# empymod/emg3d

Hardware: AMD Instinct MI355X
Metric: Mcells/s per multigrid cycle (higher is better)
Workload: dtype c128

## Files before the change

emg3d_amd/_lib.py:

```python
import ctypes
import os

import numpy as np

_HERE = os.path.dirname(os.path.abspath(__file__))
LIB_PATH = os.environ.get("EMG3D_HIP_LIB") or os.path.join(_HERE, "libemg3d_hip.so")
LAB_PATH = os.path.join(_HERE, "libemg3d_hip_lab.so")

c_i64 = ctypes.c_int64
c_int = ctypes.c_int
c_vp = ctypes.c_void_p
c_double = ctypes.c_double
c_dp = ctypes.POINTER(ctypes.c_double)

ABI_VERSION = 116

SIGNATURES = {
    "emg3d_hip_version": (c_int, []),
    "emg3d_hip_device_count": (c_int, [ctypes.POINTER(c_int)]),
    "emg3d_hip_set_device": (c_int, [c_int]),
    "emg3d_hip_device_info": (c_int, [c_int, ctypes.c_char_p, ctypes.POINTER(c_i64), ctypes.POINTER(c_int)]),
    "emg3d_hip_mem_info": (c_int, [c_int, ctypes.POINTER(c_i64), ctypes.POINTER(c_i64)]),
    "emg3d_hip_release_cached": (c_i64, []),
    "emg3d_hip_cached_bytes": (c_i64, []),
    "emg3d_hip_cached_bytes_on": (c_i64, [c_int]),
    "emg3d_mg_placement": (c_int, [c_vp, c_int, ctypes.POINTER(c_int), ctypes.POINTER(c_int), ctypes.POINTER(ctypes.c_float)]),
    "emg3d_amat_x": (c_int, [c_int, c_i64, c_i64, c_i64, c_vp, c_vp, c_vp, c_vp, c_vp, c_vp, c_vp, c_vp, c_vp]),
    "emg3d_get_h_field": (c_int, [c_int, c_i64, c_i64, c_i64, c_vp, c_vp, c_vp, c_vp, c_vp, c_vp, c_double, c_double]),
    "emg3d_gauss_seidel": (c_int, [c_int, c_int, c_i64, c_i64, c_i64, c_vp, c_vp, c_vp, c_vp, c_vp, c_vp,
                                   c_vp, c_vp, c_vp, c_int, c_int]),
    "emg3d_restrict": (c_int, [c_int, c_i64, c_i64, c_i64, c_i64, c_i64, c_i64, c_vp, c_vp, c_vp, c_int]),
    "emg3d_restrict_weights": (c_int, [c_vp, c_vp, c_vp, c_i64, c_vp, c_vp, c_vp, c_i64, c_vp, c_vp, c_vp]),
    "emg3d_solve": (c_int, [c_int, c_vp, c_vp, c_i64]),
    "emg3d_blocks_to_amat": (c_int, [c_int, c_vp, c_vp, c_i64, c_vp, c_vp, c_vp, c_i64, c_i64]),
    "emg3d_prolongation": (c_int, [c_int, c_i64, c_i64, c_i64, c_vp, c_vp, c_vp, c_vp, c_vp, c_vp, c_int]),
    "emg3d_restrict_model": (c_int, [c_int, c_i64, c_i64, c_i64, c_vp, c_vp, c_int]),
    "emg3d_sweep_plan": (c_int, [c_int, c_i64, c_i64, c_i64, c_int, c_int, c_int, c_int, ctypes.c_char_p, ctypes.POINTER(c_i64)]),
    "emg3d_sweep_thm_zkeep": (c_int, [c_int, c_i64, c_i64, c_i64, c_int, c_int, c_int, c_int, ctypes.POINTER(c_i64)]),
    "emg3d_sweep_fuse_plan": (c_int, [c_int, c_i64, c_i64, c_i64, c_int, c_int, c_int, c_int, c_int, c_int, c_int, c_i64, ctypes.POINTER(c_i64),
                                      ctypes.POINTER(c_i64), c_i64]),
    "emg3d_mg_create": (c_int, [ctypes.POINTER(c_vp), c_int, c_i64, c_i64, c_i64, c_vp, c_vp, c_vp, c_vp,
                                c_vp, c_vp, c_vp, c_vp, c_int]),
    "emg3d_mg_destroy": (None, [c_vp]),
    "emg3d_mg_create_sv": (c_int, [ctypes.POINTER(c_vp), c_int, c_i64, c_i64, c_i64, c_vp, c_vp, c_vp, c_vp,
                                   c_vp, c_vp, c_vp, c_vp, c_double, c_double, c_int]),
    "emg3d_mg_create_vs": (c_int, [ctypes.POINTER(c_vp), c_int, c_i64, c_i64, c_i64, c_vp, c_vp, c_vp, c_vp,
                                   c_vp, c_vp, c_vp, c_vp, c_vp, c_double, c_double, c_int, c_int]),
    "emg3d_mg_create_vse": (c_int, [ctypes.POINTER(c_vp), c_int, c_i64, c_i64, c_i64, c_vp, c_vp, c_vp, c_vp,
                                    c_vp, c_vp, c_vp, c_vp, c_vp, c_vp, c_double, c_double, c_double, c_int, c_int]),
    "emg3d_mg_set_smu0_eps": (c_int, [c_vp, c_double, c_double, c_double]),
    "emg3d_mg_set_model": (c_int, [c_vp, c_int, c_vp, c_vp, c_vp]),
    "emg3d_mg_get_sigma": (c_int, [c_vp, c_int, c_vp]),
    "emg3d_mg_set_sfield_vector": (c_int, [c_vp, c_vp, c_double, c_double]),
    "emg3d_mg_set_sfield_dipole": (c_int, [c_vp, c_vp, c_vp, c_int, c_int, c_vp]),
    "emg3d_source_field": (c_int, [c_int, c_i64, c_i64, c_i64, c_vp, c_vp, c_vp, c_vp, c_vp, c_vp, c_int, c_vp, c_vp]),
# ... 52 lines not shown
    "emg3d_volume_average_adjoint": (c_int, [c_i64, c_i64, c_i64, c_vp, c_vp, c_vp, c_i64, c_i64, c_i64, c_vp, c_vp, c_vp, c_vp,
                                             c_vp, c_vp]),
    "emg3d_mg_set_model_grid": (c_int, [c_vp, c_i64, c_i64, c_i64, c_vp, c_vp, c_vp]),
    "emg3d_mg_set_regrid_factors": (c_int, [c_vp, c_vp, c_vp, c_vp, c_vp, c_vp, c_vp]),
    "emg3d_mg_grad_acc_get_model": (c_int, [c_vp, c_vp]),
    "emg3d_mg_grad_acc3_get_model": (c_int, [c_vp, c_vp, c_vp, c_vp]),
    "emg3d_interp3d_grid": (c_int, [c_int, c_i64, c_i64, c_i64, c_vp, c_vp, c_vp, c_vp, c_i64, c_vp, c_i64, c_vp, c_i64,
                                    c_vp, c_int, c_int, c_double, c_double, c_vp]),
    "emg3d_mg_set_batch": (c_int, [c_vp, c_int]),
    "emg3d_mg_get_batch": (c_int, [c_vp]),
    "emg3d_mg_select": (c_int, [c_vp, c_int]),
    "emg3d_mg_set_mask": (c_int, [c_vp, c_vp]),
    "emg3d_mg_residual_norm": (c_int, [c_vp, c_dp]),
    "emg3d_mg_sfield_norm": (c_int, [c_vp, c_dp]),
    "emg3d_mg_smooth": (c_int, [c_vp, c_int, c_int]),
    "emg3d_mg_begin": (c_int, [c_vp, c_int]),
    "emg3d_mg_set_smu0": (c_int, [c_vp, ctypes.c_double, ctypes.c_double]),
    "emg3d_mg_cycle": (c_int, [c_vp, c_int, c_int, c_dp]),
    "emg3d_mg_cycle_next": (c_int, [c_vp, c_int, c_int, c_int, c_int, c_dp]),
    "emg3d_mg_cycles": (c_int, [c_vp, c_int, c_vp, c_int, c_vp, c_int, c_vp]),
    "emg3d_mg_efield_devptr": (c_vp, [c_vp]),
    "emg3d_mg_sfield_devptr": (c_vp, [c_vp]),
    "emg3d_mg_stream": (c_vp, [c_vp]),
    "emg3d_mg_nE": (c_i64, [c_vp]),
    "emg3d_mg_sync": (c_int, [c_vp]),
    "emg3d_mg_device_bytes": (c_i64, [c_vp]),
    "emg3d_mg_time_sweep": (c_int, [c_vp, c_int, c_int, ctypes.POINTER(ctypes.c_float)]),
    "emg3d_mg_last_sweep_kernel": (c_int, [c_vp, ctypes.c_char_p]),
    "emg3d_mg_time_residual": (c_int, [c_vp, c_int, ctypes.POINTER(ctypes.c_float)]),
    "emg3d_mg_last_residual_kernel": (c_int, [c_vp, ctypes.c_char_p]),
# ... 131 lines not shown
    ranges = (c_i64 * cap)()
    check(load().emg3d_sweep_fuse_plan(dtype_code(dtype), int(vnC[0]), int(vnC[1]), int(vnC[2]), int(direction),
                                       1 if ordering == 'colour' else 0, int(nsys), int(cu_count), int(npass), int(own), int(max_seg), int(budget),
                                       info, ranges, cap), "emg3d_sweep_fuse_plan")
    out = {"fused": bool(info[0]), "axis": info[1], "nX": info[2], "own": info[3], "nslabs": info[4], "npass": info[5],
           "waves": info[6], "scratch_bytes": info[7], "slabs": []}
    if out["fused"]:
        per = 4 + 2 * int(npass)
        for k in range(info[4]):
            r = ranges[per * k:per * (k + 1)]
            out["slabs"].append({"own": (r[0], r[1]), "edges": (r[2], r[3]),
                                 "live": [(r[4 + 2 * p], r[5 + 2 * p]) for p in range(int(npass))]})
    return out


def rows_gram_plan(n_rows, n_cols):
    info = (c_i64 * 8)()
    check(load().emg3d_rows_gram_plan(int(n_rows), int(n_cols), info), "emg3d_rows_gram_plan")
    out = {"block": info[0], "kstep": info[1], "slab": info[2], "nslab": info[3], "nblocks": info[4], "njobs": info[5],
           "grid": info[6], "lds_bytes": info[7], "tile": 16, "jobs": []}
    rect = (c_i64 * 4)()
    for job in range(info[5]):
        check(load().emg3d_rows_gram_job(int(n_rows), job, rect), "emg3d_rows_gram_job")
        out["jobs"].append(tuple(rect))
    return out
```

emg3d_amd/csrc/emg3d_hip.hip:

```cpp
#include "../../include/emg3d_hip.h"

#include <cstring>
#include <new>

#include <chrono>
#include "mg.hpp"
#include "receivers.hpp"
#include "source.hpp"
#include "gradient.hpp"
#include "regrid.hpp"

#define EMG3D_HIP_VERSION EMG3D_HIP_ABI_VERSION

namespace {

template <class T>
MG<T>* as(emg3d_mg_t* mg) { return static_cast<MG<T>*>(reinterpret_cast<emg3d_mg*>(mg)); }

static int current_device() { int d = 0; if (hipGetDevice(&d) != hipSuccess) { (void)hipGetLastError(); d = 0; } return d; }

template <class T> static T scalar_of(double re, double im);
template <> double scalar_of<double>(double re, double) { return re; }
template <> c128 scalar_of<c128>(double re, double im) { return mk(re, im); }

// ... 524 lines not shown
    if (!f.fused || !ranges) return 0;
    const i64 per = 4 + 2 * (i64)npass;
    if (nranges < per * f.g.nslabs) return -2;
    for (int k = 0; k < f.g.nslabs; ++k) {
        int64_t* r = ranges + per * k;
        r[0] = fuse_x0(f.g, k); r[1] = fuse_x1(f.g, k);
        i64 a = -1, b = -1;
        for (int j = 0; j <= f.g.nX; ++j) if (fuse_owner(f.g, j) == k) { if (a < 0) a = j; b = j + 1; }
        r[2] = a; r[3] = b;
        for (int p = 0; p < npass; ++p) { r[4 + 2 * p] = fuse_lo(f.g, k, p); r[5 + 2 * p] = fuse_hi(f.g, k, p); }
    }
    return 0;
}

template <class T>
static int jvec_stage(MG<T>* m, const double* const hv[3], const double* dv[3]) {
    Level<T>& L = *m->lv0;
    double* stage = reinterpret_cast<double*>(L.r);
    const i64 n = L.nCells;
    int used = 0;
    for (int c = 0; c < 3; ++c) {
        dv[c] = nullptr;
        if (!hv[c]) continue;
        for (int q = 0; q < c; ++q) if (hv[q] == hv[c]) dv[c] = dv[q];
        if (dv[c]) continue;
        double* d = stage + (i64)used++ * n;
        HIP_TRY(hipMemcpyAsync(d, hv[c], (size_t)n * sizeof(double), hipMemcpyHostToDevice, m->stream));
        dv[c] = d;
    }
    return 0;
// ... 335 lines not shown
}

int emg3d_sweep_thm_zkeep(int dtype, int64_t nx, int64_t ny, int64_t nz, int dir, int order, int nsys, int cu_count, int64_t* info) {
    if (nx < 2 || ny < 2 || nz < 2 || dir < 1 || dir > 3 || order < 0 || order > 1 || nsys < 1 || nsys > 64 || !info) return -2;
    return dtype ? thm_zkeep_impl<c128>(nx, ny, nz, dir, order, nsys, cu_count, info)
                 : thm_zkeep_impl<double>(nx, ny, nz, dir, order, nsys, cu_count, info);
}

int emg3d_sweep_fuse_plan(int dtype, int64_t nx, int64_t ny, int64_t nz, int dir, int order, int nsys, int cu_count, int npass, int own,
                          int max_seg, int64_t budget, int64_t* info, int64_t* ranges, int64_t nranges) {
    if (nx < 2 || ny < 2 || nz < 2 || dir < 1 || dir > 3 || order < 0 || order > 1 || nsys < 1 || nsys > 64 || npass < 0 || !info) return -2;
    return dtype ? fuse_plan_impl<c128>(nx, ny, nz, dir, order, nsys, cu_count, npass, own, max_seg, budget, info, ranges, nranges)
                 : fuse_plan_impl<double>(nx, ny, nz, dir, order, nsys, cu_count, npass, own, max_seg, budget, info, ranges, nranges);
}

int emg3d_mg_create(emg3d_mg_t** out, int dtype, int64_t nx, int64_t ny, int64_t nz, const double* hx,
                    const double* hy, const double* hz, const double* origin, const void* eta_x,
                    const void* eta_y, const void* eta_z, const double* zeta, int device) {
    if (!out) return -1;
    return dtype ? create_impl<c128>(out, 1, nx, ny, nz, hx, hy, hz, origin, eta_x, eta_y, eta_z, zeta, device)
                 : create_impl<double>(out, 0, nx, ny, nz, hx, hy, hz, origin, eta_x, eta_y, eta_z, zeta, device);
}

int emg3d_mg_create_sv(emg3d_mg_t** out, int dtype, int64_t nx, int64_t ny, int64_t nz, const double* hx,
                       const double* hy, const double* hz, const double* origin, const double* sv_x,
                       const double* sv_y, const double* sv_z, const double* zeta, double smu0_re,
                       double smu0_im, int device) {
    if (!out || !sv_x) return -1;
    return dtype ? create_impl<c128>(out, 1, nx, ny, nz, hx, hy, hz, origin, sv_x, sv_y, sv_z, zeta, device, true, smu0_re, smu0_im)
                 : create_impl<double>(out, 0, nx, ny, nz, hx, hy, hz, origin, sv_x, sv_y, sv_z, zeta, device, true, smu0_re, smu0_im);
// ... 818 lines not shown
```

emg3d_amd/csrc/mg.hpp:

```cpp
#pragma once
#include <algorithm>
#include <cmath>
#include <cstdlib>
#include <cstring>
#include <map>
#include <memory>
#include <mutex>
#include <chrono>
#include <vector>

#include "common.hpp"
#include "smooth.hpp"
#include "stencil.hpp"
#include "gradient.hpp"
#include "regrid.hpp"
#include "rows.hpp"
#include "smooth_qpl.hpp"
#include "smooth_qc.hpp"
#include "smooth_thm.hpp"
#include "smooth_tha.hpp"
#include "sweep_launch.hpp"
#include "sweep_plan.hpp"

template <class T>
// ... 15 lines not shown
    T *eT = nullptr, *sT = nullptr;
    T* etaT[3] = {nullptr, nullptr, nullptr};
    double* zetaT = nullptr;
    bool sT_valid = false;
    FieldLayout flT;
    CellLayout clT;
    T *eW[2] = {nullptr, nullptr}, *sW[2] = {nullptr, nullptr};
    double* zetaW[2] = {nullptr, nullptr};
    bool sW_valid[2] = {false, false};
    int e_home = 0;
    T* fac[3] = {nullptr, nullptr, nullptr};
    void* qd[3][4] = {{nullptr, nullptr, nullptr, nullptr}, {nullptr, nullptr, nullptr, nullptr}, {nullptr, nullptr, nullptr, nullptr}};
    unsigned qdn[3][4] = {{0, 0, 0, 0}, {0, 0, 0, 0}, {0, 0, 0, 0}};
    T* fz[3] = {nullptr, nullptr, nullptr};
    i64 fz_n[3] = {0, 0, 0};
    FusePlan fuse[3];
    int fuse_key[3] = {-1, -1, -1};
    std::vector<int> passes[3];
    i64 fac_lines[3] = {0, 0, 0};
    i64 fac_mid[3] = {0, 0, 0};
    int fac_kind[3] = {0, 0, 0};
    SweepPlan plan[3];
    int plan_key[3] = {-1, -1, -1};
};

struct Transfer {
    int sc = -1;
    int co[3] = {0, 0, 0};
    double* w[3][3] = {{nullptr, nullptr, nullptr}, {nullptr, nullptr, nullptr}, {nullptr, nullptr, nullptr}};
    int* pidx[3] = {nullptr, nullptr, nullptr};
// ... 1141 lines not shown
        a.xcd = xcd_map;
        a.tile = q_tile;
        {
            const int ax[3] = {a.L, a.P, a.Q};
            a.rs.ihL = a.ih[a.L]; a.rs.ihP = a.ih[a.P]; a.rs.ihQ = a.ih[a.Q];
            a.rs.hL = a.h[a.L]; a.rs.hP = a.h[a.P]; a.rs.hQ = a.h[a.Q];
            a.rs.nL = (unsigned)a.nC[a.L]; a.rs.slot0 = 0;
            a.rs.nP = (unsigned)a.nC[a.P]; a.rs.nQ = (unsigned)a.nC[a.Q];
            a.rs.csL = (unsigned)a.cl.st[a.L]; a.rs.csP = (unsigned)a.cl.st[a.P]; a.rs.csQ = (unsigned)a.cl.st[a.Q];
            for (int c = 0; c < 3; ++c) {
                a.rs.off[c] = (unsigned)a.fl.off[ax[c]];
                for (int d = 0; d < 3; ++d) a.rs.st[c][d] = (unsigned)a.fl.st[ax[c]][ax[d]];
            }
        }
        a.qd = nullptr; a.qdn = 0;
        a.fe = nullptr; a.fnE = 0; a.fax = a.fnX = a.fown = a.fns = a.fnp = 0; a.fseq = 0;
        for (int c = 0; c < 4; ++c) { a.fqd[c] = nullptr; a.fqdn[c] = 0; }
        a.qpl = P.NW; a.qM = P.M; a.seg = P.seg; a.qlpw = 0;
        a.tha = P.helpers;
        a.mode = 0; a.cP = a.cQ = 0; a.cntA = a.cntB = 0; a.t = a.jQ0 = a.cnt = 0;
        a.bt = sweep ? batch(L) : Batch();
    }

    void ensure_factor(Level<T>& L, int dir) {
        const SweepPlan& P = plan(L, dir);
        if (P.xt) ensure_transposed_model(L);
        if (L.fac[dir]) return;
        L.fac_lines[dir] = (L.nC[dir == 0 ? 1 : 0] - 1) * (L.nC[dir == 2 ? 1 : 2] - 1);
        L.fac[dir] = dalloc<T>(L.fac_lines[dir] * P.fac_entries);
        L.fac_mid[dir] = P.mid;
        L.fac_kind[dir] = P.fac_kind;
// ... 283 lines not shown
        L.passes[dir].clear();
        if (order != 1) return F;
        colour_passes(L, dir, nu, L.passes[dir]);
        const std::vector<int>& seq = L.passes[dir];
        plan(L, dir);
        F = plan_fuse(knobs, SweepShape{{L.nC[0], L.nC[1], L.nC[2]}, (int)sizeof(T)}, dir, (int)seq.size());
        if (!F.fused) return F;
        for (int c : seq) if (!L.qd[dir][c]) { F.fused = false; return F; }
        const i64 need = (i64)nsys * F.g.nslabs * L.nE;
        if (L.fz_n[dir] < need) {
            T* z = try_alloc<T>(need);
            if (!z) { F.fused = false; return F; }
            if (L.fz[dir]) release(L.fz[dir]);
            L.fz[dir] = z; L.fz_n[dir] = need;
        }
        return F;
    }
    void smooth_fused(Level<T>& L, int dir, const SweepPlan& P, const FusePlan& F, const std::vector<int>& seq, const LineArgs<T>& a) {
        LineArgs<T> b = a;
        b.mode = 0; b.xcd = 0;
        b.fe = L.fz[dir]; b.fnE = L.nE; b.fax = F.axis;
        b.fnX = F.g.nX; b.fown = F.g.own; b.fns = F.g.nslabs; b.fnp = F.g.npass;
        b.fseq = 0;
        for (int p = 0; p < F.g.npass; ++p) b.fseq |= (unsigned long long)seq[(size_t)p] << (4 * p);
        for (int c = 0; c < 4; ++c) { b.fqd[c] = L.qd[dir][c]; b.fqdn[c] = L.qd[dir][c] ? L.qdn[dir][c] : 0u; }
        if (log_launches) fprintf(stderr, "[sweep] nC %lld %lld %lld L %d lines %lld kernel %s split %d fused passes %d slabs %d own %d\n", (long long)a.nC[0],
                                  (long long)a.nC[1], (long long)a.nC[2], a.L, (long long)a.nLinesTot, P.name, a.split, F.g.npass, F.g.nslabs, F.g.own);
        memcpy(sweep_name, P.name, sizeof sweep_name);
        if (broken) return;
        qpl_fused_launch<T>(P.family == SweepFamily::qpl_chain, bgrid((unsigned)F.g.nslabs), stream, b);
        ScatterArgs sa;
        sa.nE = L.nE; sa.g = F.g;
        int Pa, Qa;
        sweep_axes(dir, Pa, Qa);
        sa.ax = F.axis ? Qa : Pa;
        for (int c = 0; c < 3; ++c) {
            sa.off[c] = L.fl.off[c];
            sa.d0[c] = (unsigned)((c == 0) ? L.nC[0] : L.nC[0] + 1); sa.d1[c] = (unsigned)((c == 1) ? L.nC[1] : L.nC[1] + 1);
        }
        hipLaunchKernelGGL(k_scatter_slabs<T>, dim3((unsigned)((L.nE + EMG_BLOCK - 1) / EMG_BLOCK), (unsigned)nsys), dim3(EMG_BLOCK), 0, stream,
                           a.e, (const T*)L.fz[dir], sa, a.bt);
    }

    void smooth_line(Level<T>& L, int dir, int nu, bool conv_in = true, bool conv_out = true) {
        if (nu <= 0) return;
        ensure_factor(L, dir);
        ensure_qdesc(L, dir);
        const FusePlan& F = ensure_fuse(L, dir, nu);
        if (dry) { prepare_work(L, dir); return; }
        if (conv_in) to_work(L, dir);
        ensure_sflags(L, dir);
        LineArgs<T> a;
        line_args(L, dir, a, true);
        const SweepPlan& P = plan(L, dir);
        const i64 nP = L.nC[a.P], nQ = L.nC[a.Q];
        const i64 nB[2] = {(nQ - 0) / 2, (nQ - 1) / 2};
        if (order == 1) {
            if (F.fused) smooth_fused(L, dir, P, F, L.passes[dir], a);
            else for (int c : L.passes[dir]) {
                a.mode = 0; a.cP = c & 1; a.cQ = c >> 1;
                a.cntA = a.nA[a.cP]; a.cntB = nB[a.cQ];
                a.rs.slot0 = (unsigned)a.base[c];
                a.qd = L.qd[dir][c]; a.qdn = (L.qd[dir][c] ? L.qdn[dir][c] : 0u);
                launch_sweep(P, a, a.cntA * a.cntB);
            }
            nu = 0;
        }
        int iback = 0;
        for (int it = 0; it < nu; ++it) {
            iback = 1 - iback;
            {
                const i64 tmin = 3, tmax = (nP - 1) + 2 * (nQ - 1);
                if (lex_loop && a.qpl && a.qM == 1 && a.seg <= 16) {
// ... 57 lines not shown
                                       dim3(EMG_LINE_BLOCK), 0, stream, a);
                }
            }
        }
        if (hl) convert_field(L, L.eW[1], L.e, 1, true);
        check_launch();
    }

    void smoothing(Level<T>& L, int nu, int lr_dir) {
        const int lr = current_lr_dir(lr_dir, L.nC);
        if (lr == 0) smooth_point(L, nu);
        int dirs[3], nd = 0;
        if (lr == 1 || lr == 5 || lr == 6 || lr == 7) dirs[nd++] = 0;
        if (lr == 2 || lr == 4 || lr == 6 || lr == 7) dirs[nd++] = 1;
        if (lr == 3 || lr == 4 || lr == 5 || lr == 7) dirs[nd++] = 2;
        for (int k = 0; k < nd; ++k) {
            const bool in = (k == 0) || work_id(L, dirs[k - 1]) != work_id(L, dirs[k]);
            const bool out = (k == nd - 1) || work_id(L, dirs[k + 1]) != work_id(L, dirs[k]);
            smooth_line(L, dirs[k], nu, in, out);
        }
    }

    void residual(Level<T>& L, int mode, int slot) {
        ResidualArgs<T> a;
        for (int q = 0; q < 3; ++q) { a.nC[q] = L.nC[q]; a.eta[q] = L.eta[q]; a.h[q] = L.h[q]; a.ih[q] = L.ih[q]; }
        a.fl = L.fl; a.r = L.r; a.s = L.s; a.e = L.e; a.zeta = L.zeta; a.bt = batch(L);
        if (!dry && L.e_home == 1) {
            if (!L.sW_valid[1]) { convert_field(L, L.sW[1], L.s, 1, true); L.sW_valid[1] = true; }
            a.e = L.eW[1]; a.s = L.sW[1]; a.xs = 1;
        }
        const i64 plane = (L.nC[0] + 1) * (L.nC[1] + 1);
        const i64 cells = L.nC[0] * L.nC[1] * L.nC[2];
        const int kz = cells < res_zm_min ? 1 : res_kz ? res_kz : (cells * nsys >= ((i64)8 << 20) ? 8 : 4);
        const i64 nNz = L.nC[2] + 1;
// ... 209 lines not shown
```

emg3d_amd/csrc/smooth.hpp:

```cpp
#pragma once
#include "common.hpp"

#define EMG_LINE_BLOCK 64

template <class T>
struct LineArgs {
    int L, P, Q;
    i64 nC[3];
    FieldLayout fl;
    CellLayout cl;
    T* e;
    const T* s;
    const T* eta[3];
    const double* zeta;
    const double* h[3];
    const double* ih[3];
    int split;
    i64 mid;
    int xcd;
    int tile;
    struct Resolved {
        const double *ihL, *ihP, *ihQ;
        const double *hL, *hP, *hQ;
        unsigned nL, csL, csP, csQ;
// ... 2 lines not shown
        unsigned off[3], st[3][3];
    } rs;
    Batch bt;
    int qm;
    int qpl;
    int qM, seg;
    const unsigned char* sflag;
    int zsep;
    int qlpw;
    int tha;
    int fcomp;
    T* fac;
    const void* qd;
    unsigned qdn;
    T* fe;
    i64 fnE;
    int fax, fnX, fown, fns, fnp;
    unsigned long long fseq;
    const void* fqd[4];
    unsigned fqdn[4];
    i64 nLinesTot;
    i64 base[4];
    i64 nA[2];
    i64 nB2[2];
    int mode;
    int cP, cQ;
    i64 cntA, cntB;
    i64 t, jQ0, cnt;
};

// ... 1174 lines not shown
```

emg3d_amd/csrc/smooth_qpl.hpp:

```cpp
#pragma once
#include "smooth.hpp"
#include "sweep_plan.hpp"


template <int K>
__device__ __forceinline__ double quad_bcast(double v) {
    constexpr int ctrl = K | (K << 2) | (K << 4) | (K << 6);
    int lo = __double2loint(v), hi = __double2hiint(v);
    lo = __builtin_amdgcn_update_dpp(0, lo, ctrl, 0xf, 0xf, false);
    hi = __builtin_amdgcn_update_dpp(0, hi, ctrl, 0xf, 0xf, false);
    return __hiloint2double(hi, lo);
}
template <int K>
__device__ __forceinline__ c128 quad_bcast(c128 v) { return mk(quad_bcast<K>(v.re), quad_bcast<K>(v.im)); }
__device__ __forceinline__ double quad_sum(double v) {
    int lo = __double2loint(v), hi = __double2hiint(v);
    double o = __hiloint2double(__builtin_amdgcn_update_dpp(0, hi, 0xb1, 0xf, 0xf, false),
                                __builtin_amdgcn_update_dpp(0, lo, 0xb1, 0xf, 0xf, false));
    v += o;
    lo = __double2loint(v); hi = __double2hiint(v);
    o = __hiloint2double(__builtin_amdgcn_update_dpp(0, hi, 0x4e, 0xf, 0xf, false),
                         __builtin_amdgcn_update_dpp(0, lo, 0x4e, 0xf, 0xf, false));
    return v + o;
}
// ... 450 lines not shown
        }
        if (j > 0) {
            const double ar = (r == 0) ? av[j][0] : (r == 1) ? av[j][1] : (r == 2) ? av[j][2] : av[j][3];
            const double dr = (r == 0) ? dv[j][0] : (r == 1) ? dv[j][1] : (r == 2) ? dv[j][2] : dv[j][3];
            T vr = x0 * ar;
            cmac(vr, xr, dr);
            v[0] = quad_bcast<0>(vr); v[1] = quad_bcast<1>(vr); v[2] = quad_bcast<2>(vr); v[3] = quad_bcast<3>(vr);
        }
    }
    QPL_TS(6);
    };

    if constexpr (FZ) {
        const FuseGeom g{a.fnX, a.fown, a.fns, a.fnp};
        const int k = (int)wg;
        {
            T* __restrict__ dst = ebase;
            const T* __restrict__ src = a.e + boff_;
            const int ra = fuse_lo(g, k, 0) - 1, rb = fuse_hi(g, k, 0) + 1;
            const int X = a.fax ? 2 : 1;
            const u32 nO = a.fax ? a.rs.nP : a.rs.nQ;
#pragma unroll
            for (int c = 0; c < 3; ++c) {
                const u32 dL = a.rs.nL + (c != 0 ? 1u : 0u), dX = (u32)g.nX + (c != X ? 1u : 0u), dO = nO + ((c == 0 || c == X) ? 1u : 0u);
                const int rbc = rb < (int)dX - 1 ? rb : (int)dX - 1;
                if (rbc < ra) continue;
                const u32 w = (u32)(rbc - ra + 1);
                const u32 stL = a.rs.st[c][0], stX = a.fax ? a.rs.st[c][2] : a.rs.st[c][1], stO = a.fax ? a.rs.st[c][1] : a.rs.st[c][2];
                const bool xf = stX < stL;
                const u32 n0 = xf ? w : dL, n1 = xf ? dL : w, tot = n0 * n1 * dO;
                for (u32 idx = (u32)tid; idx < tot; idx += 64u * NW) {
                    const u32 t = idx / n0, i0 = idx - t * n0, i2 = t / n1, i1 = t - i2 * n1;
                    const u32 iX = (u32)ra + (xf ? i0 : i1), iL = xf ? i1 : i0;
                    const u32 off = a.rs.off[c] + iL * stL + iX * stX + i2 * stO;
                    dst[off] = src[off];
                }
            }
        }
        __threadfence_block();
        __syncthreads();
        const u32 lslot = (u32)(quad >> lseg), wslot0 = (u32)(((tid >> 6) * 16) >> lseg);
        for (int p = 0; p < g.npass; ++p) {
            const int c = (int)((a.fseq >> (4 * p)) & 3ull);
            const int cP = c & 1, cQ = c >> 1;
            const u32 cA = (u32)a.nA[cP], cB = (u32)a.nB2[cQ];
            const int cX = a.fax ? cQ : cP;
            const u32 qa = (u32)(fuse_lo(g, k, p) - cX) >> 1, qb = (u32)(fuse_hi(g, k, p) + 1 - cX) >> 1;
            const u32 nx = qb > qa ? qb - qa : 0u;
            const u32 nloc = nx * (a.fax ? cA : cB);
            qd_ = a.fqd[c]; qdn_ = a.fqdn[c];
            for (u32 base = 0; base < nloc; base += (u32)lpg) {
                if (base + wslot0 < nloc) {
                    const u32 m = base + lslot;
                    const bool lv = m < nloc;
                    const u32 mm = lv ? m : base + wslot0;
                    u32 qq, bq;
                    if (a.fax == 0) { bq = mm / nx; qq = qa + (mm - bq * nx); }
                    else { const u32 t = mm / cA; qq = mm - t * cA; bq = qa + t; }
                    const u32 gl = bq * cA + qq;
                    tix = ((gl >> (4 - lseg)) << 6) + ((((gl & ((16u >> lseg) - 1u)) << lseg) + (u32)ch) << 2) + (u32)r;
                    one(lv ? 0u : 1u, 1u, 0u, 0u);
                }
            }
            __threadfence_block();
            __syncthreads();
        }
    } else if constexpr (!HL) {
        one((u32)wg * (u32)lpg + (u32)(quad >> lseg), (u32)((a.mode == 0) ? a.cntA * a.cntB : a.cnt), (u32)a.t, (u32)a.jQ0);
#ifdef EMG3D_LAB
        if ((a.tile & 512) && blockIdx.x == 0 && threadIdx.x == 0) {
            asm volatile("s_waitcnt vmcnt(0)" ::: "memory");
            const long long tend = (long long)__builtin_readcyclecounter();
            printf("[qpl<%d,%d> seg %d lines %lld] args %lld loads issued %lld loads in + coefficients %lld forward %lld backward %lld stores issued %lld stores done %lld (cycles after entry)\n",
                   NW, M, seg, (long long)(a.cntA * a.cntB), qts[1] - qts[0], qts[2] - qts[0], qts[3] - qts[0], qts[4] - qts[0], qts[5] - qts[0], qts[6] - qts[0], tend - qts[0]);
        }
#endif
    } else {
        const int nPm = (int)a.rs.nP - 1, nQm = (int)a.rs.nQ - 1;
        const int tmin = (int)a.t, tmax = (int)a.jQ0;
        for (int th = tmin; th <= tmax; ++th) {
            const int tt = a.cnt ? tmax - (th - tmin) : th;
// ... 16 lines not shown
```

emg3d_amd/csrc/sweep_plan.hpp:

```cpp
#pragma once
#include <algorithm>
#include <cstdint>
#include <cstdio>
#include <cstdlib>

typedef int64_t i64;

#ifndef LAB_ENV
#ifdef EMG3D_LAB
inline long long lab_env_(const char* name, long long def) { const char* v = getenv(name); return v ? atoll(v) : def; }
inline int lab_env_ch_(const char* name) { const char* v = getenv(name); return v ? v[0] : 0; }
#define LAB_ENV(name, def) lab_env_(name, (long long)(def))
#define LAB_ENV_CH(name) lab_env_ch_(name)
#else
#define LAB_ENV(name, def) ((long long)(def))
#define LAB_ENV_CH(name) 0
#endif
#endif

constexpr int SWEEP_THA_LPW = 8, SWEEP_THA_RING = 8, SWEEP_THA_MAX_DYN_LDS = 140 * 1024, SWEEP_THA_STATIC_LDS = 18 * 1024;
inline i64 sweep_tha_lds_bytes(i64 nL, int tsize) {
    return (2 * SWEEP_THA_RING * 5 + 2 * ((nL + 1) / 2 + 2)) * (5 * SWEEP_THA_LPW) * (i64)tsize;
}

// ... 22 lines not shown
    int q_stages = (int)LAB_ENV("EMG3D_Q_STAGES", 0);
    int q_lpw = (int)LAB_ENV("EMG3D_Q_LPW", 0);
    int q_big_lab = (int)LAB_ENV("EMG3D_Q_BIG", 0);
    int use_qpl = (int)LAB_ENV("EMG3D_QPL", 7);
    i64 qpl_min_nl = LAB_ENV("EMG3D_QPL_MIN", 2);
    i64 qpl_max_nl = LAB_ENV("EMG3D_QPL_MAX_NL", 64);
    i64 qpl_m2_min = LAB_ENV("EMG3D_QPL_M2", 32);
    int qpl_chain_seg = (int)LAB_ENV("EMG3D_QPL_CHAIN", 4);
    i64 qpl_few_lines_env = LAB_ENV("EMG3D_QPL_FEW", 0);
    i64 qpl_max_lines = LAB_ENV("EMG3D_QPL_MAX", (i64)1 << 40);
    int use_qdesc = (int)LAB_ENV("EMG3D_QDESC", 1);
    i64 qdesc_max_threads_env = LAB_ENV("EMG3D_QDESC_MAX", 0);
    int fuse_max_seg = (int)LAB_ENV("EMG3D_QPL_FUSE", 4);
    i64 fuse_own = LAB_ENV("EMG3D_QPL_FUSE_W", 0);
    i64 fuse_max_bytes = LAB_ENV("EMG3D_QPL_FUSE_BYTES", (i64)64 << 20);
    int use_tha = (int)LAB_ENV("EMG3D_THA", 3);
    i64 tha_min_nl = LAB_ENV("EMG3D_THA_MIN", 33), tha_mid_nl = LAB_ENV("EMG3D_THA_MID", 64), tha_min_lines_env = LAB_ENV("EMG3D_THA_MIN_LINES", 0);
    i64 tha_max_nl = LAB_ENV("EMG3D_THA_MAX", 128);
    i64 tha_big_max_lines_env = LAB_ENV("EMG3D_THA_BIG_LINES", 0);
    int tha_split = (int)LAB_ENV("EMG3D_THA_SPLIT", 0);

    i64 q_min_lines() const { return q_min_lines_env > 0 ? q_min_lines_env : 8 * simds; }
    i64 twist_max_lines() const { return twist_max_lines_env > 0 ? twist_max_lines_env : q_min_lines(); }
    i64 qpl_few_lines() const { return qpl_few_lines_env > 0 ? qpl_few_lines_env : simds; }
    i64 qdesc_max_threads() const { return qdesc_max_threads_env > 0 ? qdesc_max_threads_env : (9000 * simds + 1023) / 1024; }
    i64 tha_min_lines() const { return tha_min_lines_env > 0 ? tha_min_lines_env : (1100 * simds + 1023) / 1024; }
    i64 tha_big_max_lines() const { return tha_big_max_lines_env > 0 ? tha_big_max_lines_env : (i64)SWEEP_THA_LPW * (simds / 4); }
};

struct SweepShape {
// ... 178 lines not shown
    if (P.family != SweepFamily::thm || !K.thm_lds_granted || K.thm_zkeep == 0) return 0;
    const i64 n = G.nC[dir], m = (n - 1) / 2, half = std::max(m, n - m - 2);
    const i64 room = K.lds_limit - sweep_thm_static_lds(P.inst_lpw, G.tsize);
    i64 kz = std::min(half, room / sweep_thm_keep_step_bytes(P.inst_lpw, G.tsize));
    if (K.thm_zkeep > 0) kz = std::min(kz, K.thm_zkeep);
    return std::max<i64>(kz, 0);
}

constexpr int SWEEP_FUSE_MAX_PASSES = 16;
struct FuseGeom { int nX, own, nslabs, npass; };
SWEEP_HD inline int fuse_x0(const FuseGeom& g, int k) { return 1 + k * g.own; }
SWEEP_HD inline int fuse_x1(const FuseGeom& g, int k) { const int x = 1 + (k + 1) * g.own; return (k == g.nslabs - 1 || x > g.nX) ? g.nX : x; }
SWEEP_HD inline int fuse_lo(const FuseGeom& g, int k, int p) { const int v = fuse_x0(g, k) - (g.npass - 1 - p); return v < 1 ? 1 : v; }
SWEEP_HD inline int fuse_hi(const FuseGeom& g, int k, int p) { const int v = fuse_x1(g, k) + (g.npass - 1 - p); return v > g.nX - 1 ? g.nX - 1 : v; }
SWEEP_HD inline int fuse_owner(const FuseGeom& g, int j) { const int k = j <= 0 ? 0 : (j - 1) / g.own; return k > g.nslabs - 1 ? g.nslabs - 1 : k; }

struct FusePlan {
    bool fused = false;
    int axis = 0;
    int nw = 0;
    FuseGeom g = {0, 0, 0, 0};
    i64 scratch_bytes = 0;
};
inline void sweep_axes(int dir, int& P, int& Q) { P = dir == 0 ? 1 : 0; Q = dir == 2 ? 1 : 2; }
inline FusePlan plan_fuse(const SweepKnobs& K, const SweepShape& G, int dir, int npass) {
    FusePlan f;
    const SweepPlan p = plan_sweep(K, G, dir);
    if (K.order != 1 || (p.family != SweepFamily::qpl && p.family != SweepFamily::qpl_chain) || p.NW != 1 || p.M != 1 || !p.qdesc) return f;
    if (p.seg > K.fuse_max_seg || p.seg > 8 || npass < 3 || npass > SWEEP_FUSE_MAX_PASSES) return f;
#ifndef EMG3D_LAB
    if (p.family != SweepFamily::qpl_chain) return f;
#endif
    int P, Q;
    sweep_axes(dir, P, Q);
    f.axis = G.nC[Q] > G.nC[P] ? 1 : 0;
    const i64 nX = G.nC[f.axis ? Q : P];
    if (nX < 2 || nX > (1 << 20)) return f;
    i64 own = K.fuse_own > 0 ? K.fuse_own : 2;
    own = std::min<i64>(own, nX - 1);
    f.g.nX = (int)nX; f.g.own = (int)own; f.g.nslabs = (int)((nX - 1 + own - 1) / own); f.g.npass = npass;
    f.nw = p.family == SweepFamily::qpl_chain ? 8 : 4;
    f.scratch_bytes = (i64)K.nsys * f.g.nslabs * G.edges() * (i64)G.tsize;
    f.fused = f.scratch_bytes <= K.fuse_max_bytes;
    return f;
}
```

emg3d_amd/solver.py:

```python
import ctypes
import itertools
import time
from dataclasses import dataclass
from datetime import datetime, timedelta

import warnings

import numpy as np
import scipy.sparse.linalg as ssl

from emg3d_amd import _lib, core, fields, meshes, models

__all__ = ['solve', 'multigrid', 'krylov', 'smoothing', 'restriction', 'prolongation',
           'residual', 'MGParameters', 'DeviceMG', 'FrequencyHandles']

ORDERINGS = {'lex': 0, 'colour': 1, 'color': 1}


def _cells(a, dtype=np.float64):
    return np.ascontiguousarray(np.asarray(a, dtype=dtype).ravel(order='F'))


class DeviceMG:

# ... 511 lines not shown
        n = self.nsys
        out = np.empty(n, dtype=np.float64)
        _lib.check(fn(self._h, *args, out.ctypes.data_as(ctypes.POINTER(ctypes.c_double))), name)
        return float(out[0]) if n == 1 else out

    def residual_norm(self):
        return self._norms(self._lib.emg3d_mg_residual_norm, "emg3d_mg_residual_norm")

    def sfield_norm(self):
        v = ctypes.c_double()
        _lib.check(self._lib.emg3d_mg_sfield_norm(self._h, ctypes.byref(v)), "emg3d_mg_sfield_norm")
        return v.value

    def smooth(self, nu, lr_dir):
        _lib.check(self._lib.emg3d_mg_smooth(self._h, int(nu), int(lr_dir)), "emg3d_mg_smooth")

    def begin(self, sc_dir):
        _lib.check(self._lib.emg3d_mg_begin(self._h, int(sc_dir)), "emg3d_mg_begin")

    def cycle(self, sc_dir, lr_dir, nxt=None):
        if nxt is not None:
            return self._norms(self._lib.emg3d_mg_cycle_next, "emg3d_mg_cycle_next", int(sc_dir), int(lr_dir),
                               int(nxt[0]), int(nxt[1]))
        return self._norms(self._lib.emg3d_mg_cycle, "emg3d_mg_cycle", int(sc_dir), int(lr_dir))

    def cycles(self, n, sc_cycle, lr_cycle):
        sc = np.ascontiguousarray(sc_cycle, dtype=np.int32)
        lr = np.ascontiguousarray(lr_cycle, dtype=np.int32)
        ns = self.nsys
        out = np.empty(n * ns, dtype=np.float64)
# ... 1776 lines not shown
```

include/emg3d_hip.h:

```cpp
#ifndef EMG3D_HIP_H
#define EMG3D_HIP_H

#include <stdint.h>

#ifdef __cplusplus
extern "C" {
#endif

#define EMG3D_HIP_ABI_VERSION 116
int emg3d_hip_version(void);
int emg3d_hip_device_count(int* count);
int emg3d_hip_set_device(int device);
int emg3d_hip_device_info(int device, char* name, int64_t* total_mem, int* cu_count);
int emg3d_hip_mem_info(int device, int64_t* free_bytes, int64_t* total_bytes);

int64_t emg3d_hip_release_cached(void);
int64_t emg3d_hip_cached_bytes(void);
int64_t emg3d_hip_cached_bytes_on(int device);


int emg3d_amat_x(int dtype, int64_t nx, int64_t ny, int64_t nz, void* r, const void* e,
                 const void* eta_x, const void* eta_y, const void* eta_z, const double* zeta,
                 const double* hx, const double* hy, const double* hz);

// ... 20 lines not shown

int emg3d_prolongation(int dtype, int64_t nx, int64_t ny, int64_t nz, const double* hx,
                       const double* hy, const double* hz, const double* origin, void* e,
                       const void* ce, int sc_dir);

int emg3d_restrict_model(int is_complex, int64_t nx, int64_t ny, int64_t nz, void* cparam,
                         const void* param, int sc_dir);

int emg3d_sweep_plan(int dtype, int64_t nx, int64_t ny, int64_t nz, int dir, int order, int nsys, int cu_count, char* name,
                     int64_t* info);

int emg3d_sweep_thm_zkeep(int dtype, int64_t nx, int64_t ny, int64_t nz, int dir, int order, int nsys, int cu_count, int64_t* info);

int emg3d_sweep_fuse_plan(int dtype, int64_t nx, int64_t ny, int64_t nz, int dir, int order, int nsys, int cu_count, int npass, int own,
                          int max_seg, int64_t budget, int64_t* info, int64_t* ranges, int64_t nranges);

typedef struct emg3d_mg emg3d_mg_t;

int emg3d_mg_create(emg3d_mg_t** out, int dtype, int64_t nx, int64_t ny, int64_t nz,
                    const double* hx, const double* hy, const double* hz, const double* origin,
                    const void* eta_x, const void* eta_y, const void* eta_z, const double* zeta,
                    int device);
int emg3d_mg_create_sv(emg3d_mg_t** out, int dtype, int64_t nx, int64_t ny, int64_t nz, const double* hx,
                       const double* hy, const double* hz, const double* origin, const double* sv_x,
                       const double* sv_y, const double* sv_z, const double* zeta, double smu0_re,
                       double smu0_im, int device);

int emg3d_mg_create_vs(emg3d_mg_t** out, int dtype, int64_t nx, int64_t ny, int64_t nz, const double* hx,
                       const double* hy, const double* hz, const double* origin, const double* sigma_x,
                       const double* sigma_y, const double* sigma_z, const double* vol, const double* zeta,
// ... 99 lines not shown
int emg3d_mg_grad_acc3_get_model(emg3d_mg_t* mg, double* out_x, double* out_y, double* out_z);
int emg3d_interp3d_grid(int dtype, int64_t nx, int64_t ny, int64_t nz, const double* px, const double* py, const double* pz,
                        const void* values, int64_t mx, const double* xi_x, int64_t my, const double* xi_y, int64_t mz,
                        const double* xi_z, int method, int has_fill, double fill_value, double cval, void* out);

int emg3d_mg_set_batch(emg3d_mg_t* mg, int n);
int emg3d_mg_get_batch(emg3d_mg_t* mg);
int emg3d_mg_select(emg3d_mg_t* mg, int b);
int emg3d_mg_set_mask(emg3d_mg_t* mg, const int* active);

int emg3d_mg_residual_norm(emg3d_mg_t* mg, double* l2);
int emg3d_mg_sfield_norm(emg3d_mg_t* mg, double* l2);

int emg3d_mg_smooth(emg3d_mg_t* mg, int nu, int lr_dir);

int emg3d_mg_set_smu0(emg3d_mg_t* mg, double smu0_re, double smu0_im);
int emg3d_mg_set_smu0_eps(emg3d_mg_t* mg, double smu0_re, double smu0_im, double seps0);

int emg3d_mg_set_model(emg3d_mg_t* mg, int map, const double* p_x, const double* p_y, const double* p_z);
int emg3d_mg_get_sigma(emg3d_mg_t* mg, int comp, double* out);

int emg3d_mg_begin(emg3d_mg_t* mg, int sc_dir);

int emg3d_mg_cycle(emg3d_mg_t* mg, int sc_dir, int lr_dir, double* l2);
int emg3d_mg_cycle_next(emg3d_mg_t* mg, int sc_dir, int lr_dir, int next_sc_dir, int next_lr_dir, double* l2);
int emg3d_mg_set_trace(emg3d_mg_t* mg, int on);
int emg3d_mg_get_trace(emg3d_mg_t* mg, int max_recs, int64_t* recs, double* norms, int* count);
int emg3d_mg_prepare(emg3d_mg_t* mg, int sc_dir, int lr_dir);

int emg3d_mg_cycles(emg3d_mg_t* mg, int ncycles, const int* sc_cycle, int n_sc, const int* lr_cycle,
// ... 41 lines not shown
```

Before: 259.2.

## Pair consecutive fused line sweeps through a ping-pong array to skip scatter pass

When two consecutive fused line-relaxation directions work on the same array, the first fused kernel now writes its owned slab region directly into a ping-pong buffer, and the second reads from that buffer and writes back into the field. This skips the separate scatter kernel launch and the scratch-to-field copy for each paired call. It costs an extra field-sized allocation and an extra owned-range copy inside the fused kernel. It also adds a planning helper and debug/introspection entry points.

```diff
diff --git a/emg3d_amd/_lib.py b/emg3d_amd/_lib.py
--- a/emg3d_amd/_lib.py
+++ b/emg3d_amd/_lib.py
@@ -13,7 +13,7 @@
 c_double = ctypes.c_double
 c_dp = ctypes.POINTER(ctypes.c_double)
 
-ABI_VERSION = 116
+ABI_VERSION = 117
 
 SIGNATURES = {
     "emg3d_hip_version": (c_int, []),
@@ -39,6 +39,8 @@
     "emg3d_sweep_thm_zkeep": (c_int, [c_int, c_i64, c_i64, c_i64, c_int, c_int, c_int, c_int, ctypes.POINTER(c_i64)]),
     "emg3d_sweep_fuse_plan": (c_int, [c_int, c_i64, c_i64, c_i64, c_int, c_int, c_int, c_int, c_int, c_int, c_int, c_i64, ctypes.POINTER(c_i64),
                                       ctypes.POINTER(c_i64), c_i64]),
+    "emg3d_sweep_fuse_pairs": (c_int, [c_int, ctypes.POINTER(c_int), ctypes.POINTER(c_int), c_int, c_int, ctypes.POINTER(c_int)]),
+    "emg3d_sweep_fuse_owned": (c_int, [c_int, c_int, c_int, ctypes.POINTER(c_i64)]),
     "emg3d_mg_create": (c_int, [ctypes.POINTER(c_vp), c_int, c_i64, c_i64, c_i64, c_vp, c_vp, c_vp, c_vp,
                                 c_vp, c_vp, c_vp, c_vp, c_int]),
     "emg3d_mg_destroy": (None, [c_vp]),
@@ -121,6 +123,7 @@
     "emg3d_mg_residual_norm": (c_int, [c_vp, c_dp]),
     "emg3d_mg_sfield_norm": (c_int, [c_vp, c_dp]),
     "emg3d_mg_smooth": (c_int, [c_vp, c_int, c_int]),
+    "emg3d_mg_fuse_roles": (c_int, [c_vp, c_int, c_int, ctypes.POINTER(c_int), ctypes.POINTER(c_int)]),
     "emg3d_mg_begin": (c_int, [c_vp, c_int]),
     "emg3d_mg_set_smu0": (c_int, [c_vp, ctypes.c_double, ctypes.c_double]),
     "emg3d_mg_cycle": (c_int, [c_vp, c_int, c_int, c_dp]),
@@ -282,6 +285,20 @@
     return out
 
 
+def sweep_fuse_pairs(fused, work_id, write_back=None, have_pingpong=True):
+    n = len(fused)
+    f, w, role = (c_int * max(n, 1))(*[int(bool(v)) for v in fused]), (c_int * max(n, 1))(*[int(v) for v in work_id]), (c_int * max(n, 1))()
+    check(load().emg3d_sweep_fuse_pairs(n, f, w, -1 if write_back is None else int(bool(write_back)), int(bool(have_pingpong)), role),
+          "emg3d_sweep_fuse_pairs")
+    return list(role[:n])
+
+
+def sweep_fuse_owned(nX, own, nslabs):
+    ranges = (c_i64 * (2 * int(nslabs)))()
+    check(load().emg3d_sweep_fuse_owned(int(nX), int(own), int(nslabs), ranges), "emg3d_sweep_fuse_owned")
+    return [(ranges[2 * k], ranges[2 * k + 1]) for k in range(int(nslabs))]
+
+
 def rows_gram_plan(n_rows, n_cols):
     info = (c_i64 * 8)()
     check(load().emg3d_rows_gram_plan(int(n_rows), int(n_cols), info), "emg3d_rows_gram_plan")
diff --git a/emg3d_amd/csrc/emg3d_hip.hip b/emg3d_amd/csrc/emg3d_hip.hip
--- a/emg3d_amd/csrc/emg3d_hip.hip
+++ b/emg3d_amd/csrc/emg3d_hip.hip
@@ -562,6 +562,28 @@
 }
 
 template <class T>
+static int fuse_roles_impl(MG<T>* m, int nu, int lr_dir, int* role, int* fused) {
+    HIP_TRY(hipSetDevice(m->device));
+    Level<T>& L = *m->lv0;
+    const int lr = current_lr_dir(lr_dir, L.nC);
+    int dirs[3], nd = 0, r[3] = {0, 0, 0};
+    for (int d = 0; d < 3; ++d) {
+        role[d] = -1; fused[d] = 0;
+        if (lr && MG<T>::lr_has(lr, d)) dirs[nd++] = d;
+    }
+    m->fuse_roles(L, dirs, nd, nu, r);
+    for (int k = 0; k < nd; ++k) {
+        const int d = dirs[k];
+        role[d] = r[k];
+        if (m->order != 1 || nu <= 0) continue;
+        m->ensure_factor(L, d);
+        m->ensure_qdesc(L, d);
+        fused[d] = m->ensure_fuse(L, d, nu).fused ? 1 : 0;
+    }
+    return finish(m);
+}
+
+template <class T>
 static int jvec_stage(MG<T>* m, const double* const hv[3], const double* dv[3]) {
     Level<T>& L = *m->lv0;
     double* stage = reinterpret_cast<double*>(L.r);
@@ -927,6 +949,31 @@
                  : fuse_plan_impl<double>(nx, ny, nz, dir, order, nsys, cu_count, npass, own, max_seg, budget, info, ranges, nranges);
 }
 
+int emg3d_sweep_fuse_pairs(int n, const int* fused, const int* work_id, int wb, int have_pingpong, int* role) {
+    if (n < 0 || n > 3 || (n > 0 && (!fused || !work_id || !role))) return -2;
+    SweepKnobs K;
+    if (wb >= 0) K.fuse_wb = wb ? 1 : 0;
+    FuseCall calls[3];
+    for (int k = 0; k < n; ++k) {
+        if (work_id[k] < 0 || work_id[k] > 5) return -2;
+        calls[k] = FuseCall{fused[k] != 0, work_id[k]};
+    }
+    plan_fuse_pairs(K, calls, n, have_pingpong != 0, role);
+    return 0;
+}
+
+int emg3d_sweep_fuse_owned(int nX, int own, int nslabs, int64_t* ranges) {
+    if (nX < 2 || own < 1 || nslabs < 1 || !ranges) return -2;
+    const FuseGeom g{nX, own, nslabs, 0};
+    for (int k = 0; k < nslabs; ++k) { ranges[2 * k] = fuse_own_lo(g, k); ranges[2 * k + 1] = fuse_own_hi(g, k); }
+    return 0;
+}
+
+int emg3d_mg_fuse_roles(emg3d_mg_t* mg, int nu, int lr_dir, int* role, int* fused) {
+    if (lr_dir < 0 || lr_dir > 7 || nu < 0 || !role || !fused) return -2;
+    DISPATCH(mg, return fuse_roles_impl<T>(m, nu, lr_dir, role, fused));
+}
+
 int emg3d_mg_create(emg3d_mg_t** out, int dtype, int64_t nx, int64_t ny, int64_t nz, const double* hx,
                     const double* hy, const double* hz, const double* origin, const void* eta_x,
                     const void* eta_y, const void* eta_z, const double* zeta, int device) {
diff --git a/emg3d_amd/csrc/mg.hpp b/emg3d_amd/csrc/mg.hpp
--- a/emg3d_amd/csrc/mg.hpp
+++ b/emg3d_amd/csrc/mg.hpp
@@ -53,6 +53,8 @@
     unsigned qdn[3][4] = {{0, 0, 0, 0}, {0, 0, 0, 0}, {0, 0, 0, 0}};
     T* fz[3] = {nullptr, nullptr, nullptr};
     i64 fz_n[3] = {0, 0, 0};
+    T* fpp = nullptr;
+    i64 fpp_n = 0;
     FusePlan fuse[3];
     int fuse_key[3] = {-1, -1, -1};
     std::vector<int> passes[3];
@@ -1224,7 +1226,7 @@
             }
         }
         a.qd = nullptr; a.qdn = 0;
-        a.fe = nullptr; a.fnE = 0; a.fax = a.fnX = a.fown = a.fns = a.fnp = 0; a.fseq = 0;
+        a.fe = nullptr; a.fout = nullptr; a.fnE = 0; a.fax = a.fnX = a.fown = a.fns = a.fnp = 0; a.fseq = 0;
         for (int c = 0; c < 4; ++c) { a.fqd[c] = nullptr; a.fqdn[c] = 0; }
         a.qpl = P.NW; a.qM = P.M; a.seg = P.seg; a.qlpw = 0;
         a.tha = P.helpers;
@@ -1538,21 +1540,44 @@
             if (L.fz[dir]) release(L.fz[dir]);
             L.fz[dir] = z; L.fz_n[dir] = need;
         }
+        if (knobs.fuse_wb && L.fpp_n < (i64)nsys * L.nE) {
+            T* z = try_alloc<T>((i64)nsys * L.nE);
+            if (z) {
+                if (L.fpp) release(L.fpp);
+                L.fpp = z; L.fpp_n = (i64)nsys * L.nE;
+            }
+        }
         return F;
     }
-    void smooth_fused(Level<T>& L, int dir, const SweepPlan& P, const FusePlan& F, const std::vector<int>& seq, const LineArgs<T>& a) {
+    void fuse_roles(Level<T>& L, const int* dirs, int nd, int nu, int* role) {
+        FuseCall calls[3];
+        for (int k = 0; k < nd; ++k) {
+            role[k] = 0;
+            calls[k] = FuseCall{false, work_id(L, dirs[k])};
+            if (order != 1 || nu <= 0 || nd < 2) continue;
+            ensure_factor(L, dirs[k]);
+            ensure_qdesc(L, dirs[k]);
+            calls[k].fused = ensure_fuse(L, dirs[k], nu).fused;
+        }
+        if (order == 1 && nu > 0 && nd >= 2) plan_fuse_pairs(knobs, calls, nd, L.fpp != nullptr && L.fpp_n >= (i64)nsys * L.nE, role);
+    }
+    void smooth_fused(Level<T>& L, int dir, const SweepPlan& P, const FusePlan& F, const std::vector<int>& seq, const LineArgs<T>& a, int wb) {
         LineArgs<T> b = a;
         b.mode = 0; b.xcd = 0;
         b.fe = L.fz[dir]; b.fnE = L.nE; b.fax = F.axis;
+        if (wb && (!L.fpp || L.fpp_n < (i64)nsys * L.nE || L.fpp == a.e)) { fprintf(stderr, "emg3d_hip: paired fused call without its ping-pong array\n"); abort(); }
+        if (wb == 1) b.fout = L.fpp;
+        else if (wb == 2) { b.e = L.fpp; b.fout = a.e; }
         b.fnX = F.g.nX; b.fown = F.g.own; b.fns = F.g.nslabs; b.fnp = F.g.npass;
         b.fseq = 0;
         for (int p = 0; p < F.g.npass; ++p) b.fseq |= (unsigned long long)seq[(size_t)p] << (4 * p);
         for (int c = 0; c < 4; ++c) { b.fqd[c] = L.qd[dir][c]; b.fqdn[c] = L.qd[dir][c] ? L.qdn[dir][c] : 0u; }
-        if (log_launches) fprintf(stderr, "[sweep] nC %lld %lld %lld L %d lines %lld kernel %s split %d fused passes %d slabs %d own %d\n", (long long)a.nC[0],
-                                  (long long)a.nC[1], (long long)a.nC[2], a.L, (long long)a.nLinesTot, P.name, a.split, F.g.npass, F.g.nslabs, F.g.own);
+        if (log_launches) fprintf(stderr, "[sweep] nC %lld %lld %lld L %d lines %lld kernel %s split %d fused passes %d slabs %d own %d write-back %d\n", (long long)a.nC[0],
+                                  (long long)a.nC[1], (long long)a.nC[2], a.L, (long long)a.nLinesTot, P.name, a.split, F.g.npass, F.g.nslabs, F.g.own, wb);
         memcpy(sweep_name, P.name, sizeof sweep_name);
         if (broken) return;
         qpl_fused_launch<T>(P.family == SweepFamily::qpl_chain, bgrid((unsigned)F.g.nslabs), stream, b);
+        if (wb) return;
         ScatterArgs sa;
         sa.nE = L.nE; sa.g = F.g;
         int Pa, Qa;
@@ -1566,7 +1591,7 @@
                            a.e, (const T*)L.fz[dir], sa, a.bt);
     }
 
-    void smooth_line(Level<T>& L, int dir, int nu, bool conv_in = true, bool conv_out = true) {
+    void smooth_line(Level<T>& L, int dir, int nu, bool conv_in = true, bool conv_out = true, int wb = 0) {
         if (nu <= 0) return;
         ensure_factor(L, dir);
         ensure_qdesc(L, dir);
@@ -1580,7 +1605,8 @@
         const i64 nP = L.nC[a.P], nQ = L.nC[a.Q];
         const i64 nB[2] = {(nQ - 0) / 2, (nQ - 1) / 2};
         if (order == 1) {
-            if (F.fused) smooth_fused(L, dir, P, F, L.passes[dir], a);
+            if (wb && !F.fused) { fprintf(stderr, "emg3d_hip: a call that is not fused was paired\n"); abort(); }
+            if (F.fused) smooth_fused(L, dir, P, F, L.passes[dir], a, wb);
             else for (int c : L.passes[dir]) {
                 a.mode = 0; a.cP = c & 1; a.cQ = c >> 1;
                 a.cntA = a.nA[a.cP]; a.cntB = nB[a.cQ];
@@ -1668,10 +1694,12 @@
         if (lr == 1 || lr == 5 || lr == 6 || lr == 7) dirs[nd++] = 0;
         if (lr == 2 || lr == 4 || lr == 6 || lr == 7) dirs[nd++] = 1;
         if (lr == 3 || lr == 4 || lr == 5 || lr == 7) dirs[nd++] = 2;
+        int role[3] = {0, 0, 0};
+        fuse_roles(L, dirs, nd, nu, role);
         for (int k = 0; k < nd; ++k) {
             const bool in = (k == 0) || work_id(L, dirs[k - 1]) != work_id(L, dirs[k]);
             const bool out = (k == nd - 1) || work_id(L, dirs[k + 1]) != work_id(L, dirs[k]);
-            smooth_line(L, dirs[k], nu, in, out);
+            smooth_line(L, dirs[k], nu, in, out, role[k]);
         }
     }
 
diff --git a/emg3d_amd/csrc/smooth.hpp b/emg3d_amd/csrc/smooth.hpp
--- a/emg3d_amd/csrc/smooth.hpp
+++ b/emg3d_amd/csrc/smooth.hpp
@@ -40,6 +40,7 @@
     const void* qd;
     unsigned qdn;
     T* fe;
+    T* fout;
     i64 fnE;
     int fax, fnX, fown, fns, fnp;
     unsigned long long fseq;
diff --git a/emg3d_amd/csrc/smooth_qpl.hpp b/emg3d_amd/csrc/smooth_qpl.hpp
--- a/emg3d_amd/csrc/smooth_qpl.hpp
+++ b/emg3d_amd/csrc/smooth_qpl.hpp
@@ -488,29 +488,33 @@
     if constexpr (FZ) {
         const FuseGeom g{a.fnX, a.fown, a.fns, a.fnp};
         const int k = (int)wg;
-        {
-            T* __restrict__ dst = ebase;
-            const T* __restrict__ src = a.e + boff_;
-            const int ra = fuse_lo(g, k, 0) - 1, rb = fuse_hi(g, k, 0) + 1;
+        auto copy_range = [&](T* __restrict__ dst, const T* __restrict__ src, const int ra, const int rb) {
             const int X = a.fax ? 2 : 1;
             const u32 nO = a.fax ? a.rs.nP : a.rs.nQ;
+            u32 n0[3], n1[3], tot[3], s0[3], s1[3], s2[3], o[3];
 #pragma unroll
             for (int c = 0; c < 3; ++c) {
                 const u32 dL = a.rs.nL + (c != 0 ? 1u : 0u), dX = (u32)g.nX + (c != X ? 1u : 0u), dO = nO + ((c == 0 || c == X) ? 1u : 0u);
                 const int rbc = rb < (int)dX - 1 ? rb : (int)dX - 1;
-                if (rbc < ra) continue;
-                const u32 w = (u32)(rbc - ra + 1);
+                const u32 w = rbc < ra ? 0u : (u32)(rbc - ra + 1);
                 const u32 stL = a.rs.st[c][0], stX = a.fax ? a.rs.st[c][2] : a.rs.st[c][1], stO = a.fax ? a.rs.st[c][1] : a.rs.st[c][2];
                 const bool xf = stX < stL;
-                const u32 n0 = xf ? w : dL, n1 = xf ? dL : w, tot = n0 * n1 * dO;
-                for (u32 idx = (u32)tid; idx < tot; idx += 64u * NW) {
-                    const u32 t = idx / n0, i0 = idx - t * n0, i2 = t / n1, i1 = t - i2 * n1;
-                    const u32 iX = (u32)ra + (xf ? i0 : i1), iL = xf ? i1 : i0;
-                    const u32 off = a.rs.off[c] + iL * stL + iX * stX + i2 * stO;
-                    dst[off] = src[off];
-                }
-            }
-        }
+                n0[c] = xf ? w : dL; n1[c] = xf ? dL : w; tot[c] = n0[c] * n1[c] * dO;
+                s0[c] = xf ? stX : stL; s1[c] = xf ? stL : stX; s2[c] = stO;
+                o[c] = a.rs.off[c] + (u32)ra * stX;
+            }
+            const u32 e1 = tot[0], e2 = e1 + tot[1], all = e2 + tot[2];
+            for (u32 idx = (u32)tid; idx < all; idx += 64u * NW) {
+                const bool c1 = idx >= e1, c2 = idx >= e2;
+                const u32 l = idx - (c2 ? e2 : c1 ? e1 : 0u);
+                const u32 m0 = c2 ? n0[2] : c1 ? n0[1] : n0[0], m1 = c2 ? n1[2] : c1 ? n1[1] : n1[0];
+                const u32 t = l / m0, i0 = l - t * m0, i2 = t / m1, i1 = t - i2 * m1;
+                const u32 off = (c2 ? o[2] : c1 ? o[1] : o[0]) + i0 * (c2 ? s0[2] : c1 ? s0[1] : s0[0]) +
+                                i1 * (c2 ? s1[2] : c1 ? s1[1] : s1[0]) + i2 * (c2 ? s2[2] : c1 ? s2[1] : s2[0]);
+                dst[off] = src[off];
+            }
+        };
+        copy_range(ebase, a.e + boff_, fuse_lo(g, k, 0) - 1, fuse_hi(g, k, 0) + 1);
         __threadfence_block();
         __syncthreads();
         const u32 lslot = (u32)(quad >> lseg), wslot0 = (u32)(((tid >> 6) * 16) >> lseg);
@@ -539,6 +543,7 @@
             __threadfence_block();
             __syncthreads();
         }
+        if (a.fout) copy_range(a.fout + boff_, ebase, fuse_own_lo(g, k), fuse_own_hi(g, k));
     } else if constexpr (!HL) {
         one((u32)wg * (u32)lpg + (u32)(quad >> lseg), (u32)((a.mode == 0) ? a.cntA * a.cntB : a.cnt), (u32)a.t, (u32)a.jQ0);
 #ifdef EMG3D_LAB
diff --git a/emg3d_amd/csrc/sweep_plan.hpp b/emg3d_amd/csrc/sweep_plan.hpp
--- a/emg3d_amd/csrc/sweep_plan.hpp
+++ b/emg3d_amd/csrc/sweep_plan.hpp
@@ -60,6 +60,7 @@
     int fuse_max_seg = (int)LAB_ENV("EMG3D_QPL_FUSE", 4);
     i64 fuse_own = LAB_ENV("EMG3D_QPL_FUSE_W", 0);
     i64 fuse_max_bytes = LAB_ENV("EMG3D_QPL_FUSE_BYTES", (i64)64 << 20);
+    int fuse_wb = (int)LAB_ENV("EMG3D_QPL_FUSE_WB", 1);
     int use_tha = (int)LAB_ENV("EMG3D_THA", 3);
     i64 tha_min_nl = LAB_ENV("EMG3D_THA_MIN", 33), tha_mid_nl = LAB_ENV("EMG3D_THA_MID", 64), tha_min_lines_env = LAB_ENV("EMG3D_THA_MIN_LINES", 0);
     i64 tha_max_nl = LAB_ENV("EMG3D_THA_MAX", 128);
@@ -268,6 +269,8 @@
 SWEEP_HD inline int fuse_lo(const FuseGeom& g, int k, int p) { const int v = fuse_x0(g, k) - (g.npass - 1 - p); return v < 1 ? 1 : v; }
 SWEEP_HD inline int fuse_hi(const FuseGeom& g, int k, int p) { const int v = fuse_x1(g, k) + (g.npass - 1 - p); return v > g.nX - 1 ? g.nX - 1 : v; }
 SWEEP_HD inline int fuse_owner(const FuseGeom& g, int j) { const int k = j <= 0 ? 0 : (j - 1) / g.own; return k > g.nslabs - 1 ? g.nslabs - 1 : k; }
+SWEEP_HD inline int fuse_own_lo(const FuseGeom& g, int k) { return k == 0 ? 0 : 1 + k * g.own; }
+SWEEP_HD inline int fuse_own_hi(const FuseGeom& g, int k) { return k == g.nslabs - 1 ? g.nX : (k + 1) * g.own; }
 
 struct FusePlan {
     bool fused = false;
@@ -298,3 +301,17 @@
     f.fused = f.scratch_bytes <= K.fuse_max_bytes;
     return f;
 }
+
+struct FuseCall { bool fused; int work_id; };
+inline bool fuse_same_array(int wa, int wb) { return wa == wb || (wa >= 3 && wb >= 3); }
+inline bool fuse_converts_between(int wa, int wb) { return wa != wb && (wa < 3 || wb < 3); }
+inline void plan_fuse_pairs(const SweepKnobs& K, const FuseCall* calls, int n, bool have_pingpong, int* role) {
+    for (int k = 0; k < n; ++k) role[k] = 0;
+    if (!K.fuse_wb || !have_pingpong) return;
+    for (int k = 0; k + 1 < n; ++k) {
+        const FuseCall &a = calls[k], &b = calls[k + 1];
+        if (!a.fused || !b.fused || !fuse_same_array(a.work_id, b.work_id) || fuse_converts_between(a.work_id, b.work_id)) continue;
+        role[k] = 1; role[k + 1] = 2;
+        ++k;
+    }
+}
diff --git a/emg3d_amd/solver.py b/emg3d_amd/solver.py
--- a/emg3d_amd/solver.py
+++ b/emg3d_amd/solver.py
@@ -549,6 +549,11 @@
 
     def smooth(self, nu, lr_dir):
         _lib.check(self._lib.emg3d_mg_smooth(self._h, int(nu), int(lr_dir)), "emg3d_mg_smooth")
+
+    def fuse_roles(self, nu, lr_dir):
+        role, fused = (ctypes.c_int * 3)(), (ctypes.c_int * 3)()
+        _lib.check(self._lib.emg3d_mg_fuse_roles(self._h, int(nu), int(lr_dir), role, fused), "emg3d_mg_fuse_roles")
+        return [None if role[d] < 0 else (bool(fused[d]), role[d]) for d in range(3)]
 
     def begin(self, sc_dir):
         _lib.check(self._lib.emg3d_mg_begin(self._h, int(sc_dir)), "emg3d_mg_begin")
diff --git a/include/emg3d_hip.h b/include/emg3d_hip.h
--- a/include/emg3d_hip.h
+++ b/include/emg3d_hip.h
@@ -7,7 +7,7 @@
 extern "C" {
 #endif
 
-#define EMG3D_HIP_ABI_VERSION 116
+#define EMG3D_HIP_ABI_VERSION 117
 int emg3d_hip_version(void);
 int emg3d_hip_device_count(int* count);
 int emg3d_hip_set_device(int device);
@@ -58,6 +58,10 @@
 
 int emg3d_sweep_fuse_plan(int dtype, int64_t nx, int64_t ny, int64_t nz, int dir, int order, int nsys, int cu_count, int npass, int own,
                           int max_seg, int64_t budget, int64_t* info, int64_t* ranges, int64_t nranges);
+
+int emg3d_sweep_fuse_pairs(int n, const int* fused, const int* work_id, int wb, int have_pingpong, int* role);
+
+int emg3d_sweep_fuse_owned(int nX, int own, int nslabs, int64_t* ranges);
 
 typedef struct emg3d_mg emg3d_mg_t;
 
@@ -187,6 +191,8 @@
 
 int emg3d_mg_smooth(emg3d_mg_t* mg, int nu, int lr_dir);
 
+int emg3d_mg_fuse_roles(emg3d_mg_t* mg, int nu, int lr_dir, int* role, int* fused);
+
 int emg3d_mg_set_smu0(emg3d_mg_t* mg, double smu0_re, double smu0_im);
 int emg3d_mg_set_smu0_eps(emg3d_mg_t* mg, double smu0_re, double smu0_im, double seps0);
 
```

After: 260.8 (median of 6 runs). About the same (+0.6%).
